# pasensio97/SDslam

Hardware: AMD Instinct MI355X
Metric: tracked frames/sec (ORB+ImageAlign+PnP) at 640x480, 1000 kp (higher is better)
Workload: dtype u8; 1 GPU; BASELINE configs[3] at the configs[1] pyramid: 640x480, 8-level x1.2, 1000 kp; ORB extract + ImageAlign (levels 4,3,2) + SearchByProjection + PnP RANSAC (maxIts 200; iterations actually run: tracking.mean_pnp_iterations with --full); pose_solver=pnp, pyramid=8x1.2, unique_scenes=64, inputs=resident in HBM, pose_records=packed on the device every step (single GPU: no collective)

## Files before the change

include/sdslam_hip.h:

```cpp
#ifndef SDSLAM_HIP_H_
#define SDSLAM_HIP_H_

#include <stddef.h>
#include <stdint.h>

#ifdef __cplusplus
extern "C" {
#endif

#define SD_OK 0
#define SD_ERR_INVALID_ARG 1
#define SD_ERR_HIP 2
#define SD_ERR_CAPACITY 3
#define SD_ERR_NO_DEVICE 4
#define SD_FALSE 100

const char* sd_last_error(void);
int sd_device_count(void);
const char* sd_version(void);

int sd_set_option(const char* name, int value);
int sd_get_option(const char* name, int* value);
int sd_option_count(void);
const char* sd_option_name(int index);
// ... 166 lines not shown
#define SD_REFRESH_NORMAL 2
#define SD_REFRESH_SKIPPED 16
#define SD_REFRESH_NOT_RESIDENT 32
#define SD_REFRESH_TOO_MANY 64
#define SD_REFRESH_BAD_INDEX 128
int sd_track_set_observations(sd_track* h, int n_points, const int32_t* obs_off, const int32_t* obs_frame, const int32_t* obs_kp,
                              const uint8_t* obs_kf_bad, const int32_t* ref_obs, const uint8_t* point_bad);
int sd_track_refresh_points(sd_track* h, int point_row, int write_local);
int sd_track_get_refreshed(sd_track* h, uint8_t* status, int32_t* best_obs, int32_t* best_median, uint8_t* desc, double* normal,
                           float* max_dist, float* min_dist, int cap);
int sd_debug_refresh_points(int n_points, const int32_t* obs_off, const uint8_t* obs_desc, const double* obs_centre,
                            const int32_t* obs_octave, const uint8_t* obs_kf_bad, const int32_t* ref_obs, const uint8_t* point_bad,
                            const double* Xw, const float* scale_factors, int nlevels, uint8_t* status, int32_t* best_obs,
                            int32_t* best_median, uint8_t* desc, double* normal, float* max_dist, float* min_dist);

int sd_track_align(sd_track* h, int n_frames, int mode);
int sd_track_match(sd_track* h, int n_frames, float th, int mono, int check_ori);
int sd_track_pnp(sd_track* h, int n_frames, double probability, int min_inliers, int max_iterations,
                 int min_set, float epsilon, float th2, int n_iterations);
int sd_track_pnp_iterate(sd_track* h, int n_frames, int n_iterations);
int sd_track_set_matches(sd_track* h, int frame0, int n_frames, const int32_t* cur_match, int cap);

int sd_track_get_align(sd_track* h, int frame0, int n_frames, double* Tcur_cm, double* error,
                       int32_t* ok, int32_t* iters, double* chi2);
int sd_track_get_matches(sd_track* h, int frame0, int n_frames, int32_t* cur_match, int cap,
                         int32_t* n_matches);
int sd_track_get_pnp(sd_track* h, int frame0, int n_frames, float* Tcw_rowmajor, uint8_t* inliers,
                     int cap, int32_t* info8);
int sd_debug_pnp_prof(unsigned long long* out32, int reset);
int sd_debug_align_prof(unsigned long long* out16, int reset);
int sd_debug_sel_prof(unsigned long long* out64, int reset);
int sd_debug_epnp(int n, const double* Xw, const double* uv, double fx, double fy, double cx, double cy,
                  double* R9, double* t3, double* reproj_err);
int sd_track_debug_read(sd_track* h, int which, int frame, void* out, size_t bytes);
int sd_track_debug_features_in_area(sd_track* h, int frame, float x, float y, float r, int min_level, int max_level,
                                    int32_t* indices, int cap, int32_t* n_out, int32_t* grid_counts);
int sd_track_pack_records(sd_track* h, int n_frames, int source, void* d_records);

int sd_track_set_map_ids(sd_track* h, int frame0, int n_frames, int which, const int32_t* ids, int cap);
int sd_track_advance(sd_track* h, int n_frames, int source);
int sd_track_set_prior(sd_track* h, int frame0, int n_frames, const double* T_cm, int relative);
int sd_track_get_last(sd_track* h, int frame0, int n_frames, int32_t* n_last, uint8_t* valid, double* Xw, uint8_t* desc, int32_t* octave,
                      float* angle, int32_t* obs, int32_t* ids);
int sd_track_get_extractors(sd_track* h, sd_orb** cur, sd_orb** ref);
int sd_track_close_points(sd_track* h, int n_frames, int source, float th_depth);
int sd_track_get_close_points(sd_track* h, int frame0, int n_frames, int32_t* out2);

int sd_track_motion_predict(sd_track* h, int n_frames, double dt);
int sd_track_motion_update(sd_track* h, int n_frames, int source);
int sd_track_motion_restart(sd_track* h, int frame0, int n_frames);
int sd_track_get_motion(sd_track* h, int frame0, int n_frames, double* X6, double* Pdiag6, int32_t* started, double* it_time,
                        double* E_cm, double* last_pose_cm);
int sd_track_set_motion(sd_track* h, int frame0, int n_frames, const double* X6, const double* Pdiag6, const int32_t* started,
                        const double* it_time);

#define SD_SENSOR_CONSTANT_VELOCITY 0
#define SD_SENSOR_IMU 1
int sd_track_set_sensor_model(sd_track* h, int model);
int sd_track_get_sensor_model(sd_track* h, int* model);
int sd_track_set_measurements(sd_track* h, int frame0, int n_frames, const double* wa6);
int sd_track_get_imu(sd_track* h, int frame0, int n_frames, double* X16, double* P256, double* gravity3, int32_t* started, double* it_time,
                     double* last_pose_cm, double* measurements6);
int sd_track_set_imu(sd_track* h, int frame0, int n_frames, const double* X16, const double* P256, const double* gravity3,
                     const int32_t* started, const double* it_time);
int sd_track_stream_fence(sd_track* h, void* hip_stream, int direction);
int sd_track_set_profiling(sd_track* h, int on);
// ... 19 lines not shown
```

sdslam_amd/capi.py:

```python
import ctypes as C
import os

import numpy as np

_HERE = os.path.dirname(os.path.abspath(__file__))
KP_DTYPE = np.dtype([("x", "<f4"), ("y", "<f4"), ("size", "<f4"), ("angle", "<f4"),
                     ("response", "<f4"), ("octave", "<i4"), ("class_id", "<i4")])
assert KP_DTYPE.itemsize == 28

SD_OK = 0


class SdError(RuntimeError):
    def __init__(self, code, msg):
        super().__init__(f"sdslam_hip status {code}: {msg}")
        self.code = code


def lib_path() -> str:
    return os.environ.get("SD_LIB") or os.path.join(_HERE, "libsdslam_hip.so")


_I, _F, _D, _Z, _P, _S = C.c_int, C.c_float, C.c_double, C.c_size_t, C.c_void_p, C.c_char_p
_PP, _PI = C.POINTER(C.c_void_p), C.POINTER(C.c_int)
# ... 68 lines not shown
    "sd_track_sim3_iterate": (_I, [_P, _I, _I]),
    "sd_track_get_sim3": (_I, [_P, _I, _I, _P, _P, _P, _P, _P, _I, _P]),
    "sd_track_set_uright_ref": (_I, [_P, _I, _I, _P, _I]),
    "sd_track_set_f12": (_I, [_P, _I, _I, _P]),
    "sd_track_search_for_triangulation": (_I, [_P, _I, _I, _I]),
    "sd_track_get_triangulation_matches": (_I, [_P, _I, _I, _P, _I, _P, _P, _P]),
    "sd_debug_search_for_triangulation": (_I, [_I, _I, _P, _P, _P, _P, _P, _P, _P, _P, _P, _P, _P, _P, _I, _I, _P, _P]),
    "sd_track_set_tri_depth": (_I, [_P, _I, _I, _I, _P, _I]),
    "sd_track_set_tri_median_depth": (_I, [_P, _I, _I, _P]),
    "sd_track_triangulate": (_I, [_P, _I, _I]),
    "sd_track_get_triangulated": (_I, [_P, _I, _I, _P, _P, _P, _I, _P]),
    "sd_track_get_new_points": (_I, [_P, _P, _P, _P, _P, _P, _P, _P, _P, _P, _P, _I]),
    "sd_debug_triangulate": (_I, [_I, _I, _P, _P, _P, _P, _P, _P, _P, _P, _P, _P, _P, _P, _P, _P, _I, _F, _I, _F, _P, _P, _P]),
    "sd_track_set_fuse_scw": (_I, [_P, _I, _I, _P]),
    "sd_track_fuse": (_I, [_P, _I, _I, _I, _F, _I]),
    "sd_track_get_fuse": (_I, [_P, _I, _I, _P, _P, _I, _P]),
    "sd_debug_fuse": (_I, [_I, _P, _P, _P, _I, _P, _P, _P, _P, _P, _P, _P, _P, _I, _P, _P, _P, _I, _F, _F, _I, _I, _P, _P, _P, _P]),
    "sd_track_set_observations": (_I, [_P, _I, _P, _P, _P, _P, _P, _P]),
    "sd_track_refresh_points": (_I, [_P, _I, _I]),
    "sd_track_get_refreshed": (_I, [_P, _P, _P, _P, _P, _P, _P, _P, _I]),
    "sd_debug_refresh_points": (_I, [_I, _P, _P, _P, _P, _P, _P, _P, _P, _P, _I, _P, _P, _P, _P, _P, _P, _P]),
    "sd_track_align": (_I, [_P, _I, _I]),
    "sd_track_match": (_I, [_P, _I, _F, _I, _I]),
    "sd_track_pnp": (_I, [_P, _I, _D, _I, _I, _I, _F, _F, _I]),
    "sd_track_pnp_iterate": (_I, [_P, _I, _I]),
    "sd_track_set_matches": (_I, [_P, _I, _I, _P, _I]),
    "sd_track_get_align": (_I, [_P, _I, _I, _P, _P, _P, _P, _P]),
    "sd_track_get_matches": (_I, [_P, _I, _I, _P, _I, _P]),
    "sd_track_get_pnp": (_I, [_P, _I, _I, _P, _P, _I, _P]),
    "sd_debug_pnp_prof": (_I, [_P, _I]),
    "sd_debug_align_prof": (_I, [_P, _I]),
    "sd_debug_sel_prof": (_I, [_P, _I]),
    "sd_debug_epnp": (_I, [_I, _P, _P, _D, _D, _D, _D, _P, _P, _P]),
    "sd_track_debug_read": (_I, [_P, _I, _I, _P, _Z]),
    "sd_track_debug_features_in_area": (_I, [_P, _I, _F, _F, _F, _I, _I, _P, _I, _P, _P]),
    "sd_track_pack_records": (_I, [_P, _I, _I, _P]),
    "sd_track_set_map_ids": (_I, [_P, _I, _I, _I, _P, _I]),
    "sd_track_advance": (_I, [_P, _I, _I]),
    "sd_track_set_prior": (_I, [_P, _I, _I, _P, _I]),
    "sd_track_get_last": (_I, [_P, _I, _I, _P, _P, _P, _P, _P, _P, _P, _P]),
    "sd_track_get_extractors": (_I, [_P, _PP, _PP]),
    "sd_track_close_points": (_I, [_P, _I, _I, _F]),
    "sd_track_get_close_points": (_I, [_P, _I, _I, _P]),
    "sd_track_motion_predict": (_I, [_P, _I, _D]),
    "sd_track_motion_update": (_I, [_P, _I, _I]),
    "sd_track_motion_restart": (_I, [_P, _I, _I]),
    "sd_track_get_motion": (_I, [_P, _I, _I, _P, _P, _P, _P, _P, _P]),
    "sd_track_set_motion": (_I, [_P, _I, _I, _P, _P, _P, _P]),
    "sd_track_set_sensor_model": (_I, [_P, _I]),
    "sd_track_get_sensor_model": (_I, [_P, _PI]),
    "sd_track_set_measurements": (_I, [_P, _I, _I, _P]),
    "sd_track_get_imu": (_I, [_P, _I, _I, _P, _P, _P, _P, _P, _P, _P]),
    "sd_track_set_imu": (_I, [_P, _I, _I, _P, _P, _P, _P, _P]),
    "sd_track_stream_fence": (_I, [_P, _P, _I]),
    "sd_track_set_profiling": (_I, [_P, _I]),
    "sd_track_stage_ms": (_I, [_P, _P, _I]),
    "sd_track_set_next_map_id": (_I, [_P, _I, _I, _P]),
    "sd_track_stereo_init": (_I, [_P, _I, _I]),
    "sd_track_set_keyframe_state": (_I, [_P, _I, _I, _P]),
    "sd_track_need_keyframe": (_I, [_P, _I, _I, _I, _I, _I]),
    "sd_track_set_keyframe_flags": (_I, [_P, _I, _I, _P]),
    "sd_track_get_keyframe_flags": (_I, [_P, _I, _I, _P]),
    "sd_track_create_keyframe_points": (_I, [_P, _I, _I, _F, _I, _I]),
    "sd_track_get_created": (_I, [_P, _I, _I, _P, _P, _P, _P, _I]),
    "sd_hamming": (_I, [_P, _P]),
}
# ... 717 lines not shown
        _check(self.L.sd_track_get_keyframe_flags(self.h, frame0, n, _p(out)))
        return out

    def create_keyframe_points(self, n_frames, source, th_depth, use_flags=False, frame_id=0):
        _check(self.L.sd_track_create_keyframe_points(self.h, n_frames, int(source), float(th_depth), int(bool(use_flags)), int(frame_id)))

    def get_created(self, frame0, n, cap=None):
        cap = self.cap if cap is None else cap
        info = np.zeros((n, 4), np.int32)
        idx, ids, Xw = np.full((n, cap), -1, np.int32), np.full((n, cap), -1, np.int32), np.zeros((n, cap, 3))
        _check(self.L.sd_track_get_created(self.h, frame0, n, _p(info), _p(idx), _p(Xw), _p(ids), cap))
        return dict(mode=info[:, 0].copy(), created=info[:, 1].copy(), P=info[:, 2].copy(), candidates=info[:, 3].copy(), kp_index=idx,
                    Xw=Xw, ids=ids)

    def set_profiling(self, on=True):
        _check(self.L.sd_track_set_profiling(self.h, int(on)))

    def stage_ms(self):
        ms = np.zeros(3, np.float32)
        _check(self.L.sd_track_stage_ms(self.h, _p(ms), 3))
        return ms


def debug_epnp(Xw, uv, K):
    L = lib()
    Xw = np.ascontiguousarray(Xw, np.float64)
    uv = np.ascontiguousarray(uv, np.float64)
    R, t, e = np.zeros(9), np.zeros(3), C.c_double()
    _check(L.sd_debug_epnp(len(Xw), _p(Xw), _p(uv), float(K[0]), float(K[1]), float(K[2]), float(K[3]), _p(R), _p(t),
                           C.byref(e)))
    return R.reshape(3, 3), t, e.value


def debug_search_for_triangulation(kps1, desc1, has_mp1, uright1, kps2, desc2, has_mp2, uright2, F12, epipole, scale_factors,
                                   level_sigma2, check_ori=False):
    L = lib()
    k1, k2 = np.ascontiguousarray(kps1, KP_DTYPE), np.ascontiguousarray(kps2, KP_DTYPE)
    n1, n2 = len(k1), len(k2)
    d1, d2 = np.ascontiguousarray(desc1, np.uint8).reshape(n1, 32), np.ascontiguousarray(desc2, np.uint8).reshape(n2, 32)
    h1, h2 = np.ascontiguousarray(has_mp1, np.uint8), np.ascontiguousarray(has_mp2, np.uint8)
    u1, u2 = np.ascontiguousarray(uright1, np.float32), np.ascontiguousarray(uright2, np.float32)
    assert len(h1) == len(u1) == n1 and len(h2) == len(u2) == n2
    F, e = np.ascontiguousarray(F12, np.float64).reshape(9), np.ascontiguousarray(epipole, np.float32).reshape(2)
    sf, s2 = np.ascontiguousarray(scale_factors, np.float32), np.ascontiguousarray(level_sigma2, np.float32)
    assert len(sf) == len(s2)
    m, n = np.full(max(n1, 1), -1, np.int32), np.zeros(1, np.int32)
    _check(L.sd_debug_search_for_triangulation(n1, n2, _p(k1), _p(d1), _p(h1), _p(u1), _p(k2), _p(d2), _p(h2), _p(u2), _p(F), _p(e),
                                               _p(sf), _p(s2), len(sf), int(check_ori), _p(m), _p(n)))
    return int(n[0]), m[:n1]


def debug_triangulate(kps1_un, kps1, uright1, depth1, kps2_un, kps2, uright2, depth2, matches12, Tcw1, Tcw2, cam5, scale_factors,
                      level_sigma2, scale_factor, monocular=True, median_depth=-1.0):
    L = lib()
    k1u, k1 = np.ascontiguousarray(kps1_un, KP_DTYPE), np.ascontiguousarray(kps1, KP_DTYPE)
    k2u, k2 = np.ascontiguousarray(kps2_un, KP_DTYPE), np.ascontiguousarray(kps2, KP_DTYPE)
    n1, n2 = len(k1u), len(k2u)
    u1, z1 = np.ascontiguousarray(uright1, np.float32), np.ascontiguousarray(depth1, np.float32)
    u2, z2 = np.ascontiguousarray(uright2, np.float32), np.ascontiguousarray(depth2, np.float32)
    m = np.ascontiguousarray(matches12, np.int32)
    assert len(k1) == len(u1) == len(z1) == len(m) == n1 and len(k2) == len(u2) == len(z2) == n2
    T1, T2 = _cm(Tcw1), _cm(Tcw2)
    cam = np.ascontiguousarray(cam5, np.float32)
    sf, s2 = np.ascontiguousarray(scale_factors, np.float32), np.ascontiguousarray(level_sigma2, np.float32)
    assert len(cam) == 5 and len(sf) == len(s2)
    v, b, X = np.zeros(max(n1, 1), np.uint8), np.zeros(max(n1, 1), np.uint8), np.zeros((max(n1, 1), 3))
# ... 70 lines not shown
```

sdslam_amd/csrc/track.hip:

```cpp
#include <hip/hip_runtime.h>

#include <cmath>
#include <cstdlib>
#include <cstring>
#include <string>
#include <type_traits>
#include <vector>

#include "track_handle.h"

using namespace sd;

__global__ void k_pack_records(TrackBuffers tb, int source, int n_frames, double* __restrict__ out) {
  const int f = blockIdx.x * blockDim.x + threadIdx.x;
  if (f >= n_frames) return;
  double* r = out + (size_t)f * 20;
  if (source == 0) {
    const float* T = tb.pnp_T + (size_t)f * 16;
    for (int c = 0; c < 4; c++)
      for (int rr = 0; rr < 4; rr++) r[c * 4 + rr] = (double)T[rr * 4 + c];
  } else {
    const double* T = (source == 4 ? tb.Tcur : tb.po_T) + (size_t)f * 16;
    for (int i = 0; i < 16; i++) r[i] = T[i];
  }
// ... 751 lines not shown
  SD_TRY(download_rows(cur_match, cap, h->tb.cur_match, frame0, n_frames, h->kp_cap, s));
  SD_TRY(download(n_matches, h->tb.n_matches, frame0, n_frames, 1, s));
  return wait_for(s);
}

int sd_track_get_pnp(sd_track* h, int frame0, int n_frames, float* Tcw_rowmajor, uint8_t* inliers, int cap, int32_t* info8) {
  TRACK_RANGE(h, frame0, n_frames);
  SD_REQUIRE(!inliers || cap >= h->kp_cap, SD_ERR_CAPACITY, "cap smaller than the keypoint capacity");
  hipStream_t s = h->cur->stream;
  SD_TRY(download(Tcw_rowmajor, h->tb.pnp_T, frame0, n_frames, 16, s));
  SD_TRY(download_rows(inliers, cap, h->tb.pnp_inliers, frame0, n_frames, h->kp_cap, s));
  SD_TRY(download(info8, h->tb.pnp_info, frame0, n_frames, 8, s));
  return wait_for(s);
}

int sd_debug_pnp_prof(unsigned long long* out32, int reset) {
  SD_REQUIRE(out32, SD_ERR_INVALID_ARG, "null output");
  return read_pnp_prof(out32, reset);
}

int sd_debug_sel_prof(unsigned long long* out64, int reset) {
  SD_REQUIRE(out64, SD_ERR_INVALID_ARG, "null output");
  return read_sel_prof(out64, reset);
}

int sd_debug_align_prof(unsigned long long* out16, int reset) {
  SD_REQUIRE(out16, SD_ERR_INVALID_ARG, "null output");
  return read_align_prof(out16, reset);
}

int sd_debug_epnp(int n, const double* Xw, const double* uv, double fx, double fy, double cx, double cy, double* R9, double* t3,
                  double* reproj_err) {
  SD_REQUIRE(n >= 4 && Xw && uv && R9 && t3, SD_ERR_INVALID_ARG, "bad arguments");
  return run_epnp_debug(n, Xw, uv, fx, fy, cx, cy, R9, t3, reproj_err);
}

int sd_track_debug_read(sd_track* h, int which, int frame, void* out, size_t bytes) {
  SD_REQUIRE(h && out && frame >= 0 && frame < h->max_batch, SD_ERR_INVALID_ARG, "bad arguments");
  SD_REQUIRE(which != 2 || bytes <= 15 * sizeof(double), SD_ERR_CAPACITY, "the Fuse pose of a slot is 15 doubles");
  const size_t M = (size_t)h->max_points, row = (size_t)frame * M;
  const size_t lm_bytes[5] = {M * 32, M * 24, M * 4, M * 4, M * 4};
  SD_REQUIRE(which < 3 || (which <= 7 && bytes <= lm_bytes[which - 3]), SD_ERR_CAPACITY, "unknown buffer or more bytes than a local-map row holds");
  SD_HIP_CHECK(hipSetDevice(h->device));
  SD_HIP_CHECK(hipStreamSynchronize(h->pnp_stream));
  SD_HIP_CHECK(hipStreamSynchronize(h->cur->stream));
  const void* src = which == 0   ? (const void*)(h->tb.pnp_pts + (size_t)frame * h->kp_cap * 6)
                    : which == 2 ? (const void*)(h->fu.pose + (size_t)frame * 15)
                    : which == 3 ? (const void*)(h->tb.lm_desc + row * 32)
                    : which == 4 ? (const void*)(h->tb.lm_normal + row * 3)
                    : which == 5 ? (const void*)(h->tb.lm_min + row)
                    : which == 6 ? (const void*)(h->tb.lm_max + row)
                    : which == 7 ? (const void*)(h->tb.lm_mfmax + row)
                                 : (const void*)(h->tb.pnp_kpidx + (size_t)frame * h->kp_cap);
  SD_HIP_CHECK(hipMemcpy(out, src, bytes, hipMemcpyDeviceToHost));
  return SD_OK;
}

int sd_track_debug_features_in_area(sd_track* h, int frame, float x, float y, float r, int min_level, int max_level, int32_t* indices,
                                    int cap, int32_t* n_out, int32_t* grid_counts) {
  SD_TRY(check_ready(h, frame + 1, true));
  SD_REQUIRE(frame >= 0 && indices && n_out && cap >= 0, SD_ERR_INVALID_ARG, "bad arguments");
  hipStream_t s = h->pnp_stream;
  SD_TRY(wait_inputs(h, false));
  int32_t* d = nullptr;
  const size_t n_ints = (size_t)h->kp_cap + 1 + 64 * 48;
  SD_HIP_CHECK(hipMalloc(&d, n_ints * sizeof(int32_t)));
  const int rc = launch_features_in_area(h->cur, h->tb, h->cam, frame, x, y, r, min_level, max_level, d, h->kp_cap, d + h->kp_cap, d + h->kp_cap + 1, s);
// ... 73 lines not shown
```

sdslam_amd/csrc/track_internal.h:

```cpp
#pragma once
#include <hip/hip_runtime.h>
#include <stdint.h>

#include "orb_internal.h"

namespace sd {

struct TrackBuffers {
  int max_points;
  int kp_cap;
  int cur_bcast;
  uint8_t* valid;
  double* Xw;
  uint8_t* mp_desc;
  int32_t* octave;
  float* angle;
  int32_t* obs;
  int32_t* n_last;
  int32_t* last_id;
  uint8_t* valid2;
  double* Xw2;
  uint8_t* mp_desc2;
  int32_t* octave2;
  float* angle2;
// ... 210 lines not shown
                   int point_row, int write_local, hipStream_t s);
int launch_stereo_from_depth(const sd_orb* cur, const TrackBuffers& tb, const TrackCam& cam, const float* d_depth, int w, int h,
                             int stride_elems, size_t frame_stride_elems, int n_frames, hipStream_t s);
int launch_stereo_from_depth_typed(const sd_orb* cur, const TrackBuffers& tb, const TrackCam& cam, const void* d_depth, int u16,
                                   int convert, float scale, int w, int h, int stride_elems, size_t frame_stride_elems, int n_frames,
                                   hipStream_t s);
int launch_new_points(const sd_orb* cur, const TrackBuffers& tb, const TrackCam& cam, float inv_fx, float inv_fy, int n_frames, int mode,
                      int source, float th_depth, int use_flags, int frame_id, int min_keypoints, hipStream_t s);
int launch_need_keyframe(const TrackBuffers& tb, const int32_t* d_close, int n_frames, int rgbd, int frame_id, int min_frames,
                         int max_frames, hipStream_t s);
int launch_set_keyframe_state(const TrackBuffers& tb, const int32_t* staged, int frame0, int n_frames, hipStream_t s);
int launch_motion_init(const TrackBuffers& tb, int frame0, int n_frames, hipStream_t s);
int launch_motion_predict(const TrackBuffers& tb, int n_frames, double dt, hipStream_t s);
int launch_motion_update(const TrackBuffers& tb, int n_frames, int source, hipStream_t s);
int launch_imu_init(const TrackBuffers& tb, int frame0, int n_frames, int full, hipStream_t s);
int launch_imu_predict(const TrackBuffers& tb, int n_frames, double dt, hipStream_t s);
int launch_imu_update(const TrackBuffers& tb, int n_frames, int source, hipStream_t s);
int read_pnp_prof(unsigned long long* out32, int reset);
int read_sel_prof(unsigned long long* out64, int reset);
int read_align_prof(unsigned long long* out16, int reset);
int launch_pnp(const sd_orb* cur, const TrackBuffers& tb, const TrackCam& cam, const float* d_sigma2, const PnpParams& pp,
               int n_frames, hipStream_t s);

struct Sim3Params {
  int fix_scale, min_inliers;
  int n_iterations;
  int rand_per_frame;
  int resume;
};
int launch_sim3(const sd_orb* cur, const sd_orb* ref, const TrackBuffers& tb, const TrackCam& cam, const float* d_sigma2,
                const int32_t* d_max_its, const Sim3Params& sp, int n_frames, hipStream_t s);

int run_epnp_debug(int n, const double* Xw, const double* uv, double fx, double fy, double cx, double cy, double* R9, double* t3,
                   double* err);

}
```

sdslam_amd/csrc/track_pnp.hip:

```cpp
#include <hip/hip_runtime.h>

#include <algorithm>
#include <cfloat>
#include <cstdlib>

#include "orb_internal.h"
#include "sd_hypot.h"
#include "track_internal.h"
#include "track_pnp_lds.h"

namespace sd {

#define PNP_MAXN 2048
#define PNP_WORDS (PNP_MAXN / 64)
#define PNP_MAXSET 64

#ifdef SD_PNP_PROF
__device__ unsigned long long g_pnp_prof[32];
#define PROF_DECL long long _pt = clock64()
#define PROF(i)                                                                                       \
  do {                                                                                                \
    long long _n = clock64();                                                                         \
    if ((threadIdx.x & 63) == 0) atomicAdd(&g_pnp_prof[i], (unsigned long long)(_n - _pt));           \
    _pt = _n;                                                                                         \
// ... 826 lines not shown
    }
    epnp_Rt_from_abt(abt, pc0, pw0, Rv, tv);
    PROF(7);
    double sum2 = 0.0;
    for (int i = 0; i < n; i++) sum2 += epnp_reproj_term(Rv, tv, pws + 3 * i, us[2 * i], us[2 * i + 1], cam);
    err = sum2 / n;
    PROF(8);
  }
  return err;
}

template <int K, typename F>
__device__ __forceinline__ void ordered_sums(int n, ldsd* terms, ldsd* out, F&& term) {
  constexpr int KP = K | 1;
  const int lane = threadIdx.x & 63;
  double acc = 0;
  for (int base = 0; base < n; base += 64) {
    const int i = base + lane;
    if (i < n) {
      double tv[K];
      term(i, tv);
#pragma unroll
      for (int k = 0; k < K; k++) terms[lane * KP + k] = tv[k];
    }
    __syncthreads();
    const int cnt = min(64, n - base);
    if (lane < K) {
#pragma unroll 8
      for (int j = 0; j < cnt; j++) acc += terms[j * KP + lane];
    }
    __syncthreads();
  }
  if (lane < K) out[lane] = acc;
  __syncthreads();
}

template <typename TIn>
__device__ PNP_FN void epnp_refit_wave(int n, const TIn* pws, const TIn* us, const EpnpCam cam, ldsd* Rt_out, LMat ut, ldsd* scr) {
  const int lane = threadIdx.x & 63;
  ldsd* const terms = scr + pnp_lds::kTerms;
  ldsd* const mtm = scr + pnp_lds::kMtm;
  ldsd* const red = scr + pnp_lds::kRed;
  const LArr L{scr + pnp_lds::kRefitL};
  double cws[4][3], ci[9];
  auto PW = [&](int i, double* p) {
    p[0] = (double)pws[3 * i];
    p[1] = (double)pws[3 * i + 1];
    p[2] = (double)pws[3 * i + 2];
  };
  PROF_DECL;
  ordered_sums<3>(n, terms, red, [&](int i, double* tv) { PW(i, tv); });
  for (int j = 0; j < 3; j++) cws[0][j] = red[j] / n;
  ordered_sums<6>(n, terms, red, [&](int i, double* tv) {
    double pw[3];
    PW(i, pw);
    const double d0 = pw[0] - cws[0][0], d1 = pw[1] - cws[0][1], d2 = pw[2] - cws[0][2];
    tv[0] = d0 * d0; tv[1] = d0 * d1; tv[2] = d0 * d2;
    tv[3] = d1 * d1; tv[4] = d1 * d2; tv[5] = d2 * d2;
  });
  if (lane == 0) {
    const double pw0tpw0[9] = {red[0], red[1], red[2], red[1], red[3], red[4], red[2], red[4], red[5]};
    epnp_control_points(pw0tpw0, n, cws);
    epnp_cc_inverse(cws, ci);
    for (int i = 0; i < 9; i++) {
      red[16 + i] = cws[1 + i / 3][i % 3];
      red[32 + i] = ci[i];
// ... 48 lines not shown
          const double m2a = aa * (ca == 1 ? cam.fv : row[5]), m2b = ab * (cb == 1 ? cam.fv : row[5]);
          acc += has1 ? m1a * m1b : 0.0;
          acc += has2 ? m2a * m2b : 0.0;
        }
      }
    }
    if (mine) {
      mtm[ea * 12 + eb] = acc;
      mtm[eb * 12 + ea] = acc;
    }
  }
  __syncthreads();
  PROF(18);
  double rho[6];
  for (int i = lane; i < 144; i += 64) ut.row(i / 12)[i % 12] = mtm[i];
  __syncthreads();
  jacobi_sweeps12_coop(ut, lane, true, 0x3full);
  if (lane == 0) jacobi_finish12(ut);
  PROF(19);
  epnp_L_rho(ut, cws, L, rho, lane == 0);
  __syncthreads();
  PROF(20);
  if (lane < 3) {
    Rho6 rv;
    for (int i = 0; i < 6; i++) rv.r[i] = rho[i];
    Betas4 bt;
    epnp_betas(lane + 1, L, rv, bt);
    for (int i = 0; i < 4; i++) red[4 * lane + i] = bt.b[i];
  }
  __syncthreads();
  asm volatile("" ::: "memory");
  for (int i = 0; i < 12; i++) cws[i / 3][i % 3] = red[i < 3 ? 48 + i : 13 + i];
  for (int i = 0; i < 9; i++) ci[i] = red[32 + i];
  double betas3[3][4];
  for (int i = 0; i < 12; i++) betas3[i / 4][i % 4] = red[i];
  __syncthreads();
  PROF(22);
  double bestR[3][3], bestT[3], best_err = 0;
  for (int variant = 1; variant <= 3; variant++) {
    double ccs[4][3];
    epnp_ccs(ut, betas3[variant - 1], ccs);
    bool flip = false;
    auto PC = [&](int i, double* pc) {
      double a[4];
      AL(i, a);
      for (int j = 0; j < 3; j++) {
        const double x = a[0] * ccs[0][j] + a[1] * ccs[1][j] + a[2] * ccs[2][j] + a[3] * ccs[3][j];
        pc[j] = flip ? -x : x;
      }
    };
    {
      double pc_first[3];
      PC(0, pc_first);
      flip = pc_first[2] < 0.0;
    }
    double pc0[3], pw0[3], Rv[3][3], tv[3];
    ordered_sums<6>(n, terms, red, [&](int i, double* t6) {
      PC(i, t6);
      PW(i, t6 + 3);
    });
    for (int j = 0; j < 3; j++) {
      pc0[j] = red[j] / n;
      pw0[j] = red[3 + j] / n;
    }
    ordered_sums<9>(n, terms, red, [&](int i, double* t9) {
      double pc[3], pw[3];
      PC(i, pc);
      PW(i, pw);
      for (int j = 0; j < 3; j++) {
        t9[3 * j] = (pc[j] - pc0[j]) * (pw[0] - pw0[0]);
        t9[3 * j + 1] = (pc[j] - pc0[j]) * (pw[1] - pw0[1]);
        t9[3 * j + 2] = (pc[j] - pc0[j]) * (pw[2] - pw0[2]);
      }
    });
    if (lane == 0) {
      double abt[9];
      for (int i = 0; i < 9; i++) abt[i] = red[i];
      epnp_Rt_from_abt(abt, pc0, pw0, Rv, tv);
      for (int i = 0; i < 9; i++) red[16 + i] = Rv[i / 3][i % 3];
      for (int i = 0; i < 3; i++) red[25 + i] = tv[i];
    }
    __syncthreads();
    for (int i = 0; i < 9; i++) Rv[i / 3][i % 3] = red[16 + i];
    for (int i = 0; i < 3; i++) tv[i] = red[25 + i];
    PROF(23);
    ordered_sums<1>(n, terms, red, [&](int i, double* t1) {
      double pw[3];
      PW(i, pw);
      t1[0] = epnp_reproj_term(Rv, tv, pw, (double)us[2 * i], (double)us[2 * i + 1], cam);
    });
    const double err = red[0] / n;
    __syncthreads();
    PROF(24);
    if (variant == 1 || err < best_err) {
      best_err = err;
      for (int i = 0; i < 3; i++) {
        for (int j = 0; j < 3; j++) bestR[i][j] = Rv[i][j];
        bestT[i] = tv[i];
      }
    }
  }
  if (lane == 0) {
    for (int i = 0; i < 9; i++) Rt_out[i] = bestR[i / 3][i % 3];
    for (int i = 0; i < 3; i++) Rt_out[9 + i] = bestT[i];
    red[63] = best_err;
  }
  __syncthreads();
}

__device__ __forceinline__ bool pnp_is_inlier(const double* Rt, const float* q , const EpnpCam cam) {
  const float* p2 = q;
  const float* p3 = q + 2;
  const float maxErr = q[5];
  float Xc = (float)(Rt[0] * p3[0] + Rt[1] * p3[1] + Rt[2] * p3[2] + Rt[9]);
  float Yc = (float)(Rt[3] * p3[0] + Rt[4] * p3[1] + Rt[5] * p3[2] + Rt[10]);
  float invZc = (float)(1 / (Rt[6] * p3[0] + Rt[7] * p3[1] + Rt[8] * p3[2] + Rt[11]));
  double ue = cam.uc + cam.fu * Xc * invZc;
  double ve = cam.vc + cam.fv * Yc * invZc;
  float distX = (float)(p2[0] - ue);
  float distY = (float)(p2[1] - ve);
  float error2 = distX * distX + distY * distY;
  return error2 < maxErr;
}

template <bool kGeneral>
__global__ __launch_bounds__(64, 2) __attribute__((disable_tail_calls)) void k_pnp(const sd_keypoint* __restrict__ kps_all, const int32_t* __restrict__ nkp_all,
                                            TrackBuffers tb, TrackCam tcam, const float* __restrict__ sigma2, PnpParams pp,
                                            int n_frames) {
  __shared__ double s_work[pnp_lds::kWorkDoubles];
  __shared__ double s_Rt[PNP_CHUNK][12];
  __shared__ unsigned long long s_mask[PNP_CHUNK][PNP_WORDS];
  __shared__ unsigned long long s_best[PNP_WORDS], s_ref[PNP_WORDS];
  __shared__ int s_cnt[PNP_CHUNK];
  __shared__ double s_RtRef[12];
  __shared__ float s_bestT[12];
  __shared__ double s_scr[pnp_lds::kScrDoubles];
  __shared__ int s_modp[PNP_MAXSET], s_modv[PNP_MAXSET], s_draw[PNP_MAXSET];
  const int lane = threadIdx.x;
// ... 268 lines not shown
    for (int i = lane; i < N; i += 64)
      if ((s_ref[i >> 6] >> (i & 63)) & 1ull) inl_out[g_idx[i]] = 1;
    if (lane == 0) {
      for (int r = 0; r < 3; r++) {
        for (int c = 0; c < 3; c++) T_out[r * 4 + c] = (float)s_RtRef[r * 3 + c];
        T_out[r * 4 + 3] = (float)s_RtRef[9 + r];
      }
      T_out[12] = T_out[13] = T_out[14] = 0.f;
      T_out[15] = 1.f;
      info[0] = 1; info[1] = acc_cnt; info[2] = 0; info[3] = acc_iters; info[7] = 1;
    }
    return;
  }
  if (lane == 0) {
    info[2] = 1;
    info[3] = total;
  }
  if (best >= minInl) {
    for (int i = lane; i < N; i += 64)
      if ((s_best[i >> 6] >> (i & 63)) & 1ull) inl_out[g_idx[i]] = 1;
    if (lane == 0) {
      for (int r = 0; r < 3; r++) {
        for (int c = 0; c < 3; c++) T_out[r * 4 + c] = s_bestT[r * 3 + c];
        T_out[r * 4 + 3] = s_bestT[9 + r];
      }
      T_out[12] = T_out[13] = T_out[14] = 0.f;
      T_out[15] = 1.f;
      info[0] = 1;
      info[1] = best;
    }
  }
}

__global__ __launch_bounds__(64, 2) __attribute__((disable_tail_calls)) void k_epnp_debug(int n, const double* pws, const double* us, EpnpCam cam, double* out13) {
  __shared__ double s_work[pnp_lds::kWorkDoubles], s_scr[pnp_lds::kScrDoubles], s_Rt[12];
  const int lane = threadIdx.x;
  double e;
  if (n == 4) {
    double R[3][3], t[3];
    const int hyp = lane % PNP_CHUNK, variant = lane / PNP_CHUNK + 1;
    const bool active = hyp == 0 && variant <= 3;
    const LMat h_ut{LDS_PTR(s_work), hyp};
    const LArr h_L{LDS_PTR(s_scr) + pnp_lds::kL + hyp};
    const double err = epnp_minimal(
        active, variant,
        [&](int k, double* pw, double* u) {
          for (int j = 0; j < 3; j++) pw[j] = pws[3 * k + j];
          for (int j = 0; j < 2; j++) u[j] = us[2 * k + j];
        },
        cam, R, t, h_ut, h_L, LDS_PTR(s_scr), 1);
    const double e1 = __shfl(err, 0), e2 = __shfl(err, PNP_CHUNK), e3 = __shfl(err, 2 * PNP_CHUNK);
    int win = 1;
    e = e1;
    if (e2 < e) { win = 2; e = e2; }
    if (e3 < e) { win = 3; e = e3; }
    if (active && variant == win) {
      for (int i = 0; i < 9; i++) s_Rt[i] = R[i / 3][i % 3];
      for (int i = 0; i < 3; i++) s_Rt[9 + i] = t[i];
    }
    __syncthreads();
  } else {
    epnp_refit_wave(n, pws, us, cam, LDS_PTR(s_Rt), LMat{LDS_PTR(s_work), 0}, LDS_PTR(s_scr));
    e = s_scr[pnp_lds::kRed + 63];
  }
  if (lane == 0) {
    for (int i = 0; i < 12; i++) out13[i] = s_Rt[i];
    out13[12] = e;
  }
}

int run_epnp_debug(int n, const double* Xw, const double* uv, double fx, double fy, double cx, double cy, double* R9, double* t3,
                   double* err) {
  double *d_p = nullptr, *d_u = nullptr, *d_o = nullptr;
  SD_HIP_CHECK(hipMalloc(&d_p, sizeof(double) * 3 * n));
  SD_HIP_CHECK(hipMalloc(&d_u, sizeof(double) * 2 * n));
  SD_HIP_CHECK(hipMalloc(&d_o, sizeof(double) * 13));
  SD_HIP_CHECK(hipMemcpy(d_p, Xw, sizeof(double) * 3 * n, hipMemcpyHostToDevice));
  SD_HIP_CHECK(hipMemcpy(d_u, uv, sizeof(double) * 2 * n, hipMemcpyHostToDevice));
  EpnpCam cam = {fx, fy, cx, cy};
  hipLaunchKernelGGL(k_epnp_debug, dim3(1), dim3(64), 0, 0, n, d_p, d_u, cam, d_o);
  double out[13];
  SD_HIP_CHECK(hipMemcpy(out, d_o, sizeof(out), hipMemcpyDeviceToHost));
  for (int i = 0; i < 9; i++) R9[i] = out[i];
  for (int i = 0; i < 3; i++) t3[i] = out[9 + i];
  if (err) *err = out[12];
  (void)hipFree(d_p); (void)hipFree(d_u); (void)hipFree(d_o);
  return SD_OK;
}

int read_pnp_prof(unsigned long long* out32, int reset) {
#ifdef SD_PNP_PROF
  SD_HIP_CHECK(hipDeviceSynchronize());
  SD_HIP_CHECK(hipMemcpyFromSymbol(out32, HIP_SYMBOL(g_pnp_prof), 32 * sizeof(unsigned long long)));
  if (reset) {
    unsigned long long z[32] = {};
    SD_HIP_CHECK(hipMemcpyToSymbol(HIP_SYMBOL(g_pnp_prof), z, sizeof(z)));
  }
  return SD_OK;
#else
  set_error("library built without -DSD_PNP_PROF");
  return SD_ERR_INVALID_ARG;
#endif
}

int launch_pnp(const sd_orb* cur, const TrackBuffers& tb, const TrackCam& cam, const float* d_sigma2, const PnpParams& pp,
               int n_frames, hipStream_t s) {
  hipLaunchKernelGGL(pp.min_set == 4 ? k_pnp<false> : k_pnp<true>, dim3(n_frames), dim3(64), 0, s, keys_un(cur), cur->d_nout, tb, cam, d_sigma2, pp, n_frames);
  SD_HIP_CHECK(hipGetLastError());
  return SD_OK;
}

}
```

sdslam_amd/csrc/track_pnp_lds.h:

```cpp
#pragma once

#ifndef PNP_CHUNK
#define PNP_CHUNK 8
#endif

namespace sd {
namespace pnp_lds {

constexpr int kMatRow = 13;
constexpr int kMatElems = 12 * kMatRow;
constexpr int kMatW = 12;
constexpr int mat_index(int row, int k, int h) { return (row * kMatRow + k) * PNP_CHUNK + (int)((unsigned)(h + row) % PNP_CHUNK); }
constexpr int kWorkDoubles = PNP_CHUNK * kMatElems;

constexpr int kMrows = PNP_CHUNK * 4 * 24;
constexpr int kPark = 0, kParkSize = PNP_CHUNK * 16;
constexpr int kLElems = 60, kLSize = kLElems * PNP_CHUNK;
constexpr int kL = kPark + kParkSize;
constexpr int kTerms = 0, kTermsSize = 64 * 9;
constexpr int kMtm = kTerms + kTermsSize, kMtmSize = 144;
constexpr int kRed = kMtm + kMtmSize, kRedSize = 64;
constexpr int kRefitL = kTerms;
constexpr int kRefitScr = kRed + kRedSize;
constexpr int kScrDoubles = kMrows > kRefitScr ? kMrows : kRefitScr;
static_assert(kL + kLSize <= kMrows, "park + L reuse the M-row area");
static_assert(kRefitL >= kTerms && kRefitL + kLSize <= kTerms + kTermsSize, "the refit's L lies inside the (then idle) terms area");
static_assert(kRefitL + kLSize <= kMtm && kMtm + kMtmSize <= kRed, "the refit's L, mtm and red do not overlap");

}
}
```

Baseline: 240,600 frames/s.

## Evaluate the three EPnP beta variants concurrently across wave lanes in refit

Measured after the change: 241,400 frames/s (median of 6 runs). About the same (+0.3%).

```diff
diff --git a/include/sdslam_hip.h b/include/sdslam_hip.h
--- a/include/sdslam_hip.h
+++ b/include/sdslam_hip.h
@@ -222,6 +222,8 @@
 int sd_debug_sel_prof(unsigned long long* out64, int reset);
 int sd_debug_epnp(int n, const double* Xw, const double* uv, double fx, double fy, double cx, double cy,
                   double* R9, double* t3, double* reproj_err);
+int sd_debug_epnp_variants(int n, const double* Xw, const double* uv, double fx, double fy, double cx, double cy,
+                           double* R9, double* t3, double* reproj_err, double* errs3, int32_t* winner, int32_t* flips3);
 int sd_track_debug_read(sd_track* h, int which, int frame, void* out, size_t bytes);
 int sd_track_debug_features_in_area(sd_track* h, int frame, float x, float y, float r, int min_level, int max_level,
                                     int32_t* indices, int cap, int32_t* n_out, int32_t* grid_counts);
diff --git a/sdslam_amd/capi.py b/sdslam_amd/capi.py
--- a/sdslam_amd/capi.py
+++ b/sdslam_amd/capi.py
@@ -124,6 +124,7 @@
     "sd_debug_align_prof": (_I, [_P, _I]),
     "sd_debug_sel_prof": (_I, [_P, _I]),
     "sd_debug_epnp": (_I, [_I, _P, _P, _D, _D, _D, _D, _P, _P, _P]),
+    "sd_debug_epnp_variants": (_I, [_I, _P, _P, _D, _D, _D, _D, _P, _P, _P, _P, _P, _P]),
     "sd_track_debug_read": (_I, [_P, _I, _I, _P, _Z]),
     "sd_track_debug_features_in_area": (_I, [_P, _I, _F, _F, _F, _I, _I, _P, _I, _P, _P]),
     "sd_track_pack_records": (_I, [_P, _I, _I, _P]),
@@ -907,6 +908,17 @@
     return R.reshape(3, 3), t, e.value
 
 
+def debug_epnp_variants(Xw, uv, K):
+    L = lib()
+    Xw = np.ascontiguousarray(Xw, np.float64)
+    uv = np.ascontiguousarray(uv, np.float64)
+    R, t, e = np.zeros(9), np.zeros(3), C.c_double()
+    errs, win, flips = np.zeros(3), C.c_int32(), np.zeros(3, np.int32)
+    _check(L.sd_debug_epnp_variants(len(Xw), _p(Xw), _p(uv), float(K[0]), float(K[1]), float(K[2]), float(K[3]), _p(R), _p(t),
+                                    C.byref(e), _p(errs), C.byref(win), _p(flips)))
+    return R.reshape(3, 3), t, e.value, errs, win.value, flips
+
+
 def debug_search_for_triangulation(kps1, desc1, has_mp1, uright1, kps2, desc2, has_mp2, uright2, F12, epipole, scale_factors,
                                    level_sigma2, check_ori=False):
     L = lib()
diff --git a/sdslam_amd/csrc/track.hip b/sdslam_amd/csrc/track.hip
--- a/sdslam_amd/csrc/track.hip
+++ b/sdslam_amd/csrc/track.hip
@@ -807,7 +807,13 @@
 int sd_debug_epnp(int n, const double* Xw, const double* uv, double fx, double fy, double cx, double cy, double* R9, double* t3,
                   double* reproj_err) {
   SD_REQUIRE(n >= 4 && Xw && uv && R9 && t3, SD_ERR_INVALID_ARG, "bad arguments");
-  return run_epnp_debug(n, Xw, uv, fx, fy, cx, cy, R9, t3, reproj_err);
+  return run_epnp_debug(n, Xw, uv, fx, fy, cx, cy, R9, t3, reproj_err, nullptr, nullptr, nullptr);
+}
+
+int sd_debug_epnp_variants(int n, const double* Xw, const double* uv, double fx, double fy, double cx, double cy, double* R9,
+                           double* t3, double* reproj_err, double* errs3, int32_t* winner, int32_t* flips3) {
+  SD_REQUIRE(n >= 4 && Xw && uv && R9 && t3 && errs3 && winner && flips3, SD_ERR_INVALID_ARG, "bad arguments");
+  return run_epnp_debug(n, Xw, uv, fx, fy, cx, cy, R9, t3, reproj_err, errs3, winner, flips3);
 }
 
 int sd_track_debug_read(sd_track* h, int which, int frame, void* out, size_t bytes) {
diff --git a/sdslam_amd/csrc/track_internal.h b/sdslam_amd/csrc/track_internal.h
--- a/sdslam_amd/csrc/track_internal.h
+++ b/sdslam_amd/csrc/track_internal.h
@@ -266,6 +266,6 @@
                 const int32_t* d_max_its, const Sim3Params& sp, int n_frames, hipStream_t s);
 
 int run_epnp_debug(int n, const double* Xw, const double* uv, double fx, double fy, double cx, double cy, double* R9, double* t3,
-                   double* err);
-
-}
+                   double* err, double* errs3, int32_t* winner, int32_t* flips3);
+
+}
diff --git a/sdslam_amd/csrc/track_pnp.hip b/sdslam_amd/csrc/track_pnp.hip
--- a/sdslam_amd/csrc/track_pnp.hip
+++ b/sdslam_amd/csrc/track_pnp.hip
@@ -882,6 +882,35 @@
     __syncthreads();
   }
   if (lane < K) out[lane] = acc;
+  __syncthreads();
+}
+
+template <int K, typename F>
+__device__ __forceinline__ void ordered_sums3(int n, ldsd* terms, ldsd* out, F&& term) {
+  static_assert(K <= pnp_lds::kTailMaxK, "term rows");
+  constexpr int W = pnp_lds::kTailW;
+  const int lane = threadIdx.x & 63;
+  const int r = lane % W;
+  const bool evals = lane < pnp_lds::kTailLanes, adds = lane < 3 * K;
+  const ldsd* const mine = terms + pnp_lds::tail_term_index(lane % K, adds ? (lane / K) * W : 0);
+  double acc = 0;
+  for (int base = 0; base < n; base += W) {
+    const int i = base + r;
+    if (evals && i < n) {
+      double tv[K];
+      term(i, tv);
+#pragma unroll
+      for (int k = 0; k < K; k++) terms[pnp_lds::tail_term_index(k, lane)] = tv[k];
+    }
+    __syncthreads();
+    const int cnt = min(W, n - base);
+    if (adds) {
+#pragma unroll 7
+      for (int j = 0; j < cnt; j++) acc += mine[j];
+    }
+    __syncthreads();
+  }
+  if (adds) out[lane] = acc;
   __syncthreads();
 }
 
@@ -996,78 +1025,84 @@
   asm volatile("" ::: "memory");
   for (int i = 0; i < 12; i++) cws[i / 3][i % 3] = red[i < 3 ? 48 + i : 13 + i];
   for (int i = 0; i < 9; i++) ci[i] = red[32 + i];
-  double betas3[3][4];
-  for (int i = 0; i < 12; i++) betas3[i / 4][i % 4] = red[i];
+  const int v = min(lane / pnp_lds::kTailW, 2);
+  const bool lead = lane < pnp_lds::kTailLanes && lane % pnp_lds::kTailW == 0;
+  ldsd* const sums = scr + pnp_lds::kTailSums;
+  ldsd* const rt = scr + pnp_lds::kTailRt + 12 * v;
+  PROF(22);
+  double ccs[4][3];
+  {
+    double betas[4];
+    for (int i = 0; i < 4; i++) betas[i] = red[4 * v + i];
+    epnp_ccs(ut, betas, ccs);
+  }
+  bool flip = false;
+  auto PC = [&](int i, double* pc) {
+    double a[4];
+    AL(i, a);
+    for (int j = 0; j < 3; j++) {
+      const double x = a[0] * ccs[0][j] + a[1] * ccs[1][j] + a[2] * ccs[2][j] + a[3] * ccs[3][j];
+      pc[j] = flip ? -x : x;
+    }
+  };
+  {
+    double pc_first[3];
+    PC(0, pc_first);
+    flip = pc_first[2] < 0.0;
+  }
+  double pc0[3], pw0[3];
+  ordered_sums3<6>(n, terms, sums, [&](int i, double* t6) {
+    PC(i, t6);
+    PW(i, t6 + 3);
+  });
+  for (int j = 0; j < 3; j++) {
+    pc0[j] = sums[6 * v + j] / n;
+    pw0[j] = sums[6 * v + 3 + j] / n;
+  }
+  ordered_sums3<9>(n, terms, sums, [&](int i, double* t9) {
+    double pc[3], pw[3];
+    PC(i, pc);
+    PW(i, pw);
+    for (int j = 0; j < 3; j++) {
+      t9[3 * j] = (pc[j] - pc0[j]) * (pw[0] - pw0[0]);
+      t9[3 * j + 1] = (pc[j] - pc0[j]) * (pw[1] - pw0[1]);
+      t9[3 * j + 2] = (pc[j] - pc0[j]) * (pw[2] - pw0[2]);
+    }
+  });
+  if (lead) {
+    double abt[9], Rl[3][3], tl[3];
+    for (int i = 0; i < 9; i++) abt[i] = sums[9 * v + i];
+    epnp_Rt_from_abt(abt, pc0, pw0, Rl, tl);
+    for (int i = 0; i < 9; i++) rt[i] = Rl[i / 3][i % 3];
+    for (int i = 0; i < 3; i++) rt[9 + i] = tl[i];
+    red[pnp_lds::kRedFlip + v] = flip ? 1.0 : 0.0;
+  }
   __syncthreads();
-  PROF(22);
-  double bestR[3][3], bestT[3], best_err = 0;
-  for (int variant = 1; variant <= 3; variant++) {
-    double ccs[4][3];
-    epnp_ccs(ut, betas3[variant - 1], ccs);
-    bool flip = false;
-    auto PC = [&](int i, double* pc) {
-      double a[4];
-      AL(i, a);
-      for (int j = 0; j < 3; j++) {
-        const double x = a[0] * ccs[0][j] + a[1] * ccs[1][j] + a[2] * ccs[2][j] + a[3] * ccs[3][j];
-        pc[j] = flip ? -x : x;
-      }
-    };
-    {
-      double pc_first[3];
-      PC(0, pc_first);
-      flip = pc_first[2] < 0.0;
-    }
-    double pc0[3], pw0[3], Rv[3][3], tv[3];
-    ordered_sums<6>(n, terms, red, [&](int i, double* t6) {
-      PC(i, t6);
-      PW(i, t6 + 3);
-    });
-    for (int j = 0; j < 3; j++) {
-      pc0[j] = red[j] / n;
-      pw0[j] = red[3 + j] / n;
-    }
-    ordered_sums<9>(n, terms, red, [&](int i, double* t9) {
-      double pc[3], pw[3];
-      PC(i, pc);
-      PW(i, pw);
-      for (int j = 0; j < 3; j++) {
-        t9[3 * j] = (pc[j] - pc0[j]) * (pw[0] - pw0[0]);
-        t9[3 * j + 1] = (pc[j] - pc0[j]) * (pw[1] - pw0[1]);
-        t9[3 * j + 2] = (pc[j] - pc0[j]) * (pw[2] - pw0[2]);
-      }
-    });
-    if (lane == 0) {
-      double abt[9];
-      for (int i = 0; i < 9; i++) abt[i] = red[i];
-      epnp_Rt_from_abt(abt, pc0, pw0, Rv, tv);
-      for (int i = 0; i < 9; i++) red[16 + i] = Rv[i / 3][i % 3];
-      for (int i = 0; i < 3; i++) red[25 + i] = tv[i];
-    }
-    __syncthreads();
-    for (int i = 0; i < 9; i++) Rv[i / 3][i % 3] = red[16 + i];
-    for (int i = 0; i < 3; i++) tv[i] = red[25 + i];
+  {
+    double Rv[3][3], tv[3];
+    for (int i = 0; i < 9; i++) Rv[i / 3][i % 3] = rt[i];
+    for (int i = 0; i < 3; i++) tv[i] = rt[9 + i];
     PROF(23);
-    ordered_sums<1>(n, terms, red, [&](int i, double* t1) {
+    ordered_sums3<1>(n, terms, sums, [&](int i, double* t1) {
       double pw[3];
       PW(i, pw);
       t1[0] = epnp_reproj_term(Rv, tv, pw, (double)us[2 * i], (double)us[2 * i + 1], cam);
     });
-    const double err = red[0] / n;
-    __syncthreads();
-    PROF(24);
-    if (variant == 1 || err < best_err) {
-      best_err = err;
-      for (int i = 0; i < 3; i++) {
-        for (int j = 0; j < 3; j++) bestR[i][j] = Rv[i][j];
-        bestT[i] = tv[i];
-      }
-    }
-  }
+  }
+  PROF(24);
   if (lane == 0) {
-    for (int i = 0; i < 9; i++) Rt_out[i] = bestR[i / 3][i % 3];
-    for (int i = 0; i < 3; i++) Rt_out[9 + i] = bestT[i];
-    red[63] = best_err;
+    const double e1 = sums[0] / n, e2 = sums[1] / n, e3 = sums[2] / n;
+    int win = 1;
+    double e = e1;
+    if (e2 < e) { win = 2; e = e2; }
+    if (e3 < e) { win = 3; e = e3; }
+    const ldsd* const best = scr + pnp_lds::kTailRt + 12 * (win - 1);
+    for (int i = 0; i < 12; i++) Rt_out[i] = best[i];
+    red[pnp_lds::kRedErr3] = e1;
+    red[pnp_lds::kRedErr3 + 1] = e2;
+    red[pnp_lds::kRedErr3 + 2] = e3;
+    red[pnp_lds::kRedWin] = (double)win;
+    red[pnp_lds::kRedErr] = e;
   }
   __syncthreads();
 }
@@ -1402,10 +1437,10 @@
   }
 }
 
-__global__ __launch_bounds__(64, 2) __attribute__((disable_tail_calls)) void k_epnp_debug(int n, const double* pws, const double* us, EpnpCam cam, double* out13) {
+__global__ __launch_bounds__(64, 2) __attribute__((disable_tail_calls)) void k_epnp_debug(int n, const double* pws, const double* us, EpnpCam cam, double* out20) {
   __shared__ double s_work[pnp_lds::kWorkDoubles], s_scr[pnp_lds::kScrDoubles], s_Rt[12];
   const int lane = threadIdx.x;
-  double e;
+  double e, ev[3], flips[3], winner;
   if (n == 4) {
     double R[3][3], t[3];
     const int hyp = lane % PNP_CHUNK, variant = lane / PNP_CHUNK + 1;
@@ -1429,31 +1464,50 @@
       for (int i = 0; i < 3; i++) s_Rt[9 + i] = t[i];
     }
     __syncthreads();
+    ev[0] = e1; ev[1] = e2; ev[2] = e3;
+    flips[0] = flips[1] = flips[2] = -1.0;
+    winner = (double)win;
   } else {
     epnp_refit_wave(n, pws, us, cam, LDS_PTR(s_Rt), LMat{LDS_PTR(s_work), 0}, LDS_PTR(s_scr));
-    e = s_scr[pnp_lds::kRed + 63];
+    const double* red = s_scr + pnp_lds::kRed;
+    e = red[pnp_lds::kRedErr];
+    for (int i = 0; i < 3; i++) {
+      ev[i] = red[pnp_lds::kRedErr3 + i];
+      flips[i] = red[pnp_lds::kRedFlip + i];
+    }
+    winner = red[pnp_lds::kRedWin];
   }
   if (lane == 0) {
-    for (int i = 0; i < 12; i++) out13[i] = s_Rt[i];
-    out13[12] = e;
+    for (int i = 0; i < 12; i++) out20[i] = s_Rt[i];
+    out20[12] = e;
+    for (int i = 0; i < 3; i++) {
+      out20[13 + i] = ev[i];
+      out20[17 + i] = flips[i];
+    }
+    out20[16] = winner;
   }
 }
 
 int run_epnp_debug(int n, const double* Xw, const double* uv, double fx, double fy, double cx, double cy, double* R9, double* t3,
-                   double* err) {
+                   double* err, double* errs3, int32_t* winner, int32_t* flips3) {
   double *d_p = nullptr, *d_u = nullptr, *d_o = nullptr;
   SD_HIP_CHECK(hipMalloc(&d_p, sizeof(double) * 3 * n));
   SD_HIP_CHECK(hipMalloc(&d_u, sizeof(double) * 2 * n));
-  SD_HIP_CHECK(hipMalloc(&d_o, sizeof(double) * 13));
+  SD_HIP_CHECK(hipMalloc(&d_o, sizeof(double) * 20));
   SD_HIP_CHECK(hipMemcpy(d_p, Xw, sizeof(double) * 3 * n, hipMemcpyHostToDevice));
   SD_HIP_CHECK(hipMemcpy(d_u, uv, sizeof(double) * 2 * n, hipMemcpyHostToDevice));
   EpnpCam cam = {fx, fy, cx, cy};
   hipLaunchKernelGGL(k_epnp_debug, dim3(1), dim3(64), 0, 0, n, d_p, d_u, cam, d_o);
-  double out[13];
+  double out[20];
   SD_HIP_CHECK(hipMemcpy(out, d_o, sizeof(out), hipMemcpyDeviceToHost));
   for (int i = 0; i < 9; i++) R9[i] = out[i];
   for (int i = 0; i < 3; i++) t3[i] = out[9 + i];
   if (err) *err = out[12];
+  for (int i = 0; i < 3; i++) {
+    if (errs3) errs3[i] = out[13 + i];
+    if (flips3) flips3[i] = (int32_t)out[17 + i];
+  }
+  if (winner) *winner = (int32_t)out[16];
   (void)hipFree(d_p); (void)hipFree(d_u); (void)hipFree(d_o);
   return SD_OK;
 }
diff --git a/sdslam_amd/csrc/track_pnp_lds.h b/sdslam_amd/csrc/track_pnp_lds.h
--- a/sdslam_amd/csrc/track_pnp_lds.h
+++ b/sdslam_amd/csrc/track_pnp_lds.h
@@ -27,5 +27,17 @@
 static_assert(kRefitL >= kTerms && kRefitL + kLSize <= kTerms + kTermsSize, "the refit's L lies inside the (then idle) terms area");
 static_assert(kRefitL + kLSize <= kMtm && kMtm + kMtmSize <= kRed, "the refit's L, mtm and red do not overlap");
 
+constexpr int kTailW = 21, kTailLanes = 3 * kTailW, kTailMaxK = 9;
+constexpr int tail_term_index(int k, int lane) { return k * kTailLanes + lane; }
+constexpr int kTailSums = kMtm, kTailSumsSize = 3 * kTailMaxK;
+constexpr int kTailRt = kTailSums + 32, kTailRtSize = 3 * 12;
+static_assert(kTailLanes <= 64 && kTerms + tail_term_index(kTailMaxK - 1, kTailLanes - 1) < kTerms + kTermsSize, "the tail's term rows fit the terms area");
+static_assert(kTailSums + kTailSumsSize <= kTailRt && kTailRt + kTailRtSize <= kMtm + kMtmSize, "the tail's sums and poses fit the (then dead) mtm area");
+constexpr int kRedFlip = 56;
+constexpr int kRedWin = 59;
+constexpr int kRedErr3 = 60;
+constexpr int kRedErr = 63;
+static_assert(kRedFlip > 50 && kRedFlip + 3 <= kRedWin && kRedWin < kRedErr3 && kRedErr3 + 3 <= kRedErr && kRedErr < kRedSize, "outcome slots lie behind the control points");
+
 }
 }
```
